# slcs-jsc/mptrac

Hardware: AMD Instinct MI355X
Metric: particle-steps/s (higher is better)
Workload: dtype f64

## Files before the change

### mptrac_amd/csrc/mphip_api.hip

```cpp
#include <hip/hip_runtime.h>
#include <dlfcn.h>
#include <unistd.h>

#include <algorithm>
#include <atomic>
#include <cmath>
#include <cstdio>
#include <cstring>
#include <string>
#include <mutex>
#include <thread>
#include <vector>

#include "mphip_kernels.hpp"
#include "mphip_metprep.hpp"

using namespace mphip;

namespace {

constexpr unsigned kAdv = MPHIP_MOD_TIMESTEPS | MPHIP_MOD_POSITION | MPHIP_MOD_ADVECT | MPHIP_MOD_POSITION2;
constexpr unsigned kAdvTurb = kAdv | MPHIP_MOD_DIFF_TURB;
constexpr unsigned kAdvDiff = kAdvTurb | MPHIP_MOD_DIFF_MESO;
constexpr unsigned kAdvTurbConvSedi = kAdvTurb | MPHIP_MOD_CONVECTION | MPHIP_MOD_SEDI;
constexpr unsigned kAdvDiffConvSedi = kAdvDiff | MPHIP_MOD_CONVECTION | MPHIP_MOD_SEDI;
constexpr unsigned kDiffConvSediOnly = MPHIP_MOD_TIMESTEPS | MPHIP_MOD_DIFF_TURB | MPHIP_MOD_DIFF_MESO | MPHIP_MOD_CONVECTION
  | MPHIP_MOD_SEDI | MPHIP_MOD_POSITION2;
constexpr unsigned kTailOnly = MPHIP_MOD_TIMESTEPS;
constexpr unsigned kBound = MPHIP_MOD_BOUND_COND | MPHIP_MOD_BOUND_COND2;
constexpr unsigned kParticleBits = 0x3fffu | MPHIP_MOD_ISOSURF | kBound | MPHIP_MOD_ISOSURF_INIT;

struct MetSlot {
  bool valid = false;
  double time = 0;
  float *f3[MPHIP_N3D] = {};
  float *f2[MPHIP_N2D] = {};
  bool has3[MPHIP_N3D] = {};
  bool has2[MPHIP_N2D] = {};
  std::vector<double> lon, lat, p;
  float ps11 = 0.f;
  double ps_min = -HUGE_VAL, pct_min = -HUGE_VAL;
  double ps_max = HUGE_VAL, pbl_min = -HUGE_VAL, pbl_max = HUGE_VAL, pel_min = -HUGE_VAL;
};

}

struct mphip_ctx {
  int device = 0;
  hipStream_t stream = nullptr;
  std::string err;
  std::mutex err_lock;

  mphip_ctl_t ctl;
  bool have_ctl = false;
  DevClim *d_clim = nullptr;
  bool have_clim = false;
  double *d_zm[MPHIP_NZM] = {};
  DevZm zm[MPHIP_NZM] = {};
  double *d_ts[MPHIP_NTR] = {};
  DevTracerSeries h_tracers = {};
  DevTracerSeries *d_tracers = nullptr;

  MetSlot slot[2];
  int flip = 0;
  MetSlot next;
  bool next_pending = false;
  hipStream_t copy_stream = nullptr;
  hipEvent_t next_ready = nullptr;
  hipEvent_t main_mark = nullptr;
  bool fuse_sort = true;
  const int *fused_perm = nullptr;
  bool fuse_quantities = true;
  bool fused_quantities = false;
  bool lazy_meteo = true;
  bool meteo_pending = false;
  bool pin_host_atm = false;
  std::vector<std::pair<uintptr_t, uintptr_t>> pinned;
  std::mutex pinned_lock;
  std::thread uploader;
  int uploader_rc = 0;
  std::atomic<bool> uploader_done{ false };
  std::string uploader_err;
  int nx = 0, ny = 0, npl = 0, coord_type = 0;
  int nml = 0;
  struct PackedGrids {
    float *wind = nullptr, *temp = nullptr, *h2o = nullptr;
    float *mlw = nullptr, *zl2 = nullptr, *pl2 = nullptr;
    f32x4 *mx = nullptr, *mx2 = nullptr;
    f32x4 *cloud = nullptr, *sfa = nullptr, *sfb = nullptr, *sfc = nullptr, *sfd = nullptr;
    f32x4 *cp2 = nullptr;
    int *ml_mono = nullptr;
    bool ml_monotonic = false;
    void release() {
      for (void *q : { (void *) wind, (void *) temp, (void *) h2o, (void *) mlw, (void *) zl2, (void *) pl2, (void *) mx,
                       (void *) mx2, (void *) cloud, (void *) sfa, (void *) sfb, (void *) sfc, (void *) sfd, (void *) cp2,
                       (void *) ml_mono })
        if (q)
          (void) hipFree(q);
      *this = PackedGrids();
    }
  };
  PackedGrids pk, pk_next;
  bool pk_next_valid = false;
  std::vector<double> h_lon, h_lat, h_p;
  double *d_axes = nullptr;
  int lut_base = 0, lut_size = 0;
  size_t axes_bytes = 0;
  bool packed_dirty = true;

  long long np = 0, ip0 = 0, np_total = 0, cap = 0;
  int nq = 0;
  double *d_arr[4 + MPHIP_NQ_MAX] = {};
  double *d_alt[4 + MPHIP_NQ_MAX] = {};
  float *d_uvwp[3] = {};
  float *d_uvwp_alt[3] = {};
  double *d_dt = nullptr;
  double *d_dt_alt = nullptr;
  uint64_t rng_ctr = 0;
  double *d_iso = nullptr, *d_iso_alt = nullptr;
  int *d_kz = nullptr, *d_kz_alt = nullptr;
  double *d_iso_ts = nullptr, *d_iso_ps = nullptr;
  int iso_n = 0;

  int *d_ext = nullptr, *d_ext_alt = nullptr;
  bool ext_identity = true;
  int locality_interval = 60;
  double *d_rec = nullptr;
  size_t rec_cap = 0;
  bool grid_records = true;
  int chain_blocks = 0;
  double *h_sums = nullptr;
  size_t h_sums_cap = 0;
  double *d_grid_kernel = nullptr;
  double *d_ana_kernel = nullptr;
  size_t ana_kernel_cap = 0;
  uint32_t *d_marks = nullptr;
  size_t marks_cap = 0;
  int *d_slot_of = nullptr;
  size_t slot_of_cap = 0;
  uint32_t *d_ana_flags = nullptr;
  int grid_nk = 0;
  bool locality_zorder = false;
  int locality_tile = 0;
  int step_blocks = 8192;
  int step_blocks_multi = 32768;
  int xcd_map = 1;
  int big_grid = 0;
  int perm_records = 1;
  void *d_prec = nullptr;
  size_t prec_cap = 0;
  int multi_step = 64;
  bool force_generic = false;
  bool compact_depo = true;
  int sort_bits = 0;
  int steps_since_resort = 1 << 30;

  uint32_t *d_keys[2] = {};
  int *d_vals[2] = {};
  uint32_t *d_counts = nullptr;
  size_t counts_cap = 0;
  int sorted_buf = -1;
  int lds_tile = 0;
  bool emit_keys = true;
  unsigned char *d_depo_busy = nullptr;
  long long depo_busy_cap = 0;
  bool depo_busy_valid = false;
  bool sort_repair = true;
  bool ahead_priority = false;
  bool stored_is_sorted = false;
  long long sorted_n = 0;
  uint32_t *rep_sk = nullptr, *rep_mk[2] = {}, *rep_fk = nullptr, *rep_tiles = nullptr, *rep_nm = nullptr;
  int *rep_si = nullptr, *rep_mi[2] = {}, *rep_fv = nullptr;
  long long rep_cap = 0;
  bool sort_ahead = true;
  bool ahead_box = true;
  hipStream_t ahead_stream = nullptr;
  hipEvent_t ahead_mark = nullptr, ahead_done = nullptr;
  uint32_t *ahead_keys[2] = {};
  int *ahead_vals[2] = {};
  uint32_t *ahead_counts = nullptr;
  size_t ahead_counts_cap = 0;
  double *ahead_dt = nullptr;
  long long ahead_cap = 0;
  bool ahead_valid = false;
  double ahead_t = 0;
  int ahead_cur = 0;

  int *d_cell = nullptr;
  double *d_sums = nullptr;
  size_t sums_cap = 0;

  int *d_cnt = nullptr;
  double *d_chemgrid = nullptr;
  bool chemgrid_ok = false;
  double h2o2_low = 0;
  double *d_photo = nullptr;
  DevPhoto photo = {};
  bool photo_have[4] = {};
  RadioQnt radio = { { -1, -1, -1, -1, -1, -1 } };
  bool radio_on = false;
  bool rdepo_on = false;
  mphip_box_t rdepo_grid = {};
  double *d_rdepo_inv = nullptr;
  size_t rdepo_ntot = 0;
  bool rdepo_have_t = false;
  double rdepo_t = 0;
  const unsigned char *depo_busy_last = nullptr;
  unsigned depo_busy_last_mask = 0;
  bool mix_exchange_levels = false;
  double *d_occ = nullptr, *h_occ = nullptr, *d_band = nullptr;
  int *d_band_cnt = nullptr;
  size_t band_cap = 0;
  int mix_band_lo = -1, mix_band_hi = -1;
  size_t cnt_cap = 0;
  int deterministic_sums = 1;
  int sum_path = 0;
  unsigned long long *d_lists = nullptr;
  size_t lists_cap = 0;

  mphip_allreduce_fn allreduce = nullptr;
  void *allreduce_user = nullptr;
  void *comm = nullptr;
  int comm_ranks = 1, comm_rank = 0;

  std::mutex prep_lock;
  hipStream_t prep_stream = nullptr;
  int prep_nx = 0, prep_ny = 0, prep_np = 0;
  float *prep_in3[MPHIP_N3D] = {}, *prep_in2[MPHIP_N2D] = {};
  float *prep_out2[MPHIP_N2D] = {};
  float *prep_z[2] = {};
  double *prep_axes = nullptr;
  int prep_profile_phase = 0;

  bool prof = false;
  std::vector<hipEvent_t> ev;
  size_t ev_used = 0;
};

namespace {

int fail(mphip_ctx *ctx, const std::string &msg) {
  if (ctx) {
    std::lock_guard<std::mutex> guard(ctx->err_lock);
    ctx->err = msg;
  }
  return 1;
}

#define HIPCHK(call)                                                                         \
  do {                                                                                       \
    hipError_t e_ = (call);                                                                  \
    if (e_ != hipSuccess)                                                                    \
      return fail(ctx, std::string(#call) + ": " + hipGetErrorString(e_));                   \
  } while (0)

template <typename T>
int dev_alloc(mphip_ctx *ctx, T **p, size_t n) {
  if (*p) {
    HIPCHK(hipFree(*p));
    *p = nullptr;
  }
  if (n) {
    HIPCHK(hipMalloc((void **) p, n * sizeof(T)));
  }
  return 0;
}

void dev_free(void *p) {
  if (p)
    (void) hipFree(p);
}

int grid_for(long long n, int block = 256, int maxb = 8192) {
  long long b = (n + block - 1) / block;
  if (b < 1)
    b = 1;
  if (b > maxb)
    b = maxb;
  return (int) b;
}

DevAtm dev_atm(const mphip_ctx *c) {
  DevAtm a;
  a.time = c->d_arr[0];
  a.p = c->d_arr[1];
  a.lon = c->d_arr[2];
  a.lat = c->d_arr[3];
  for (int iq = 0; iq < MPHIP_NQ_MAX; iq++)
    a.q[iq] = iq < c->nq ? c->d_arr[4 + iq] : nullptr;
  a.up = c->d_uvwp[0];
  a.vp = c->d_uvwp[1];
  a.wp = c->d_uvwp[2];
  a.dt = c->d_dt;
  a.ext = c->ext_identity ? nullptr : c->d_ext;
  a.iso = c->d_iso;
  a.kz = c->d_kz;
  a.iso_ts = c->d_iso_ts;
  a.iso_ps = c->d_iso_ps;
  a.iso_n = c->iso_n;
  a.perm = c->fused_perm;
  a.s_time = c->d_alt[0];
  a.s_p = c->d_alt[1];
  a.s_lon = c->d_alt[2];
  a.s_lat = c->d_alt[3];
  a.nq_perm = c->fused_perm && c->fused_quantities ? c->nq : 0;
  for (int iq = 0; iq < MPHIP_NQ_MAX; iq++)
    a.s_q[iq] = iq < c->nq ? c->d_alt[4 + iq] : nullptr;
  a.np = c->np;
  a.ip0 = c->ip0;
  a.np_total = c->np_total;
  return a;
}

DevMet dev_met(const mphip_ctx *c) {
  DevMet M;
  M.wind = c->pk.wind;
  M.temp = c->pk.temp;
  M.cloud = c->pk.cloud;
  M.mx = c->pk.mx;
  M.mx2 = c->pk.mx2;
  M.sfa = c->pk.sfa;
  M.sfb = c->pk.sfb;
  M.cp2 = c->pk.cp2;
  M.sfc = c->pk.sfc;
  M.sfd = c->pk.sfd;
  M.h2o = c->pk.h2o;
  M.mlw = c->pk.mlw;
  M.zl2 = c->pk.zl2;
  M.pl2 = c->pk.pl2;
  M.ml_monotonic = c->pk.ml_monotonic ? 1 : 0;
  for (int t = 0; t < 2; t++) {
    M.zl[t] = c->slot[t ^ c->flip].f3[MPHIP_ZETAL];
    M.pll[t] = c->slot[t ^ c->flip].f3[MPHIP_PL];
  }
  M.npl = c->nml;
  M.axes = c->d_axes;
  M.lut_base = c->lut_base;
  M.lut_size = c->lut_size;
  M.lat_x0 = c->h_lat[0];
  M.lat_inv_dx = (c->ny - 1) / (c->h_lat[c->ny - 1] - c->h_lat[0]);
  M.nx = c->nx;
  M.ny = c->ny;
  M.np = c->npl;
  M.coord_type = c->coord_type;
  M.time0 = c->slot[0 ^ c->flip].time;
  M.time1 = c->slot[1 ^ c->flip].time;
  M.inv_dtime = 1.0 / (M.time1 - M.time0);
  double latmin = c->h_lat[0], latmax = c->h_lat[0];
  for (double v : c->h_lat) {
    latmin = std::min(latmin, v);
    latmax = std::max(latmax, v);
  }
  M.latmin = latmin;
  M.latmax = latmax;
  M.local = (std::fabs(c->h_lon[c->nx - 1] - c->h_lon[0] - 360.0) >= 0.01);
  const int my = (c->ny - 1) >> 1, mp = (c->npl - 1) >> 1;
  M.lat_ascending = c->h_lat[my] < c->h_lat[my + 1];
  M.p_ascending = c->h_p[mp] < c->h_p[mp + 1];
  M.lon_first = c->h_lon[0];
  M.lon_last = c->h_lon[c->nx - 1];
  M.inv_dlon0 = 1.0 / (c->h_lon[1] - c->h_lon[0]);
  M.lat_search_max = std::nextafter(latmax, -HUGE_VAL);
  M.p_min = *std::min_element(c->h_p.begin(), c->h_p.end());
  M.p_search_max = std::nextafter(*std::max_element(c->h_p.begin(), c->h_p.end()), -HUGE_VAL);
  M.p_cmp_off = M.p_ascending ? 1 : 0;
  M.p_step = M.p_ascending ? 1 : -1;
  M.ps11[0] = c->slot[0 ^ c->flip].ps11;
  M.ps11[1] = c->slot[1 ^ c->flip].ps11;
  M.ps_skip = std::min(c->slot[0].ps_min, c->slot[1].ps_min) - 1e-6;
  M.pct_skip = std::min(c->slot[0].pct_min, c->slot[1].pct_min) - 1e-6;
  {
    const double ps_lo = std::min(c->slot[0].ps_min, c->slot[1].ps_min), ps_hi = std::max(c->slot[0].ps_max, c->slot[1].ps_max);
    const double pbl_lo = std::min(c->slot[0].pbl_min, c->slot[1].pbl_min),
                 pbl_hi = std::max(c->slot[0].pbl_max, c->slot[1].pbl_max);
    auto p1_min = [&](double trans) {
      double lo = HUGE_VAL;
      for (double pbl : { pbl_lo, pbl_hi })
        for (double ps : { ps_lo, ps_hi })
          lo = std::min(lo, pbl - trans * (ps - pbl));
      return lo;
    };
    const bool known = std::isfinite(ps_lo) && std::isfinite(ps_hi) && std::isfinite(pbl_lo) && std::isfinite(pbl_hi);
    M.turb_skip = -HUGE_VAL;
    M.conv_skip = -HUGE_VAL;
    if (known && c->have_ctl) {
      const double b = std::min({ ps_lo, pbl_lo, p1_min(c->ctl.turb_pbl_trans) });
      M.turb_skip = b - 1e-6 * std::fabs(b) - 1e-6;
      double lo = ps_lo;
// ... 1028 lines not shown
  int cur = 0, rc = 0;
  if (box && !keys_ready)
    rc = sort_keys(ctx, 0, &t_next, box);
  if (!rc && (hipEventRecord(ctx->ahead_mark, main_stream) != hipSuccess
              || hipStreamWaitEvent(ctx->ahead_stream, ctx->ahead_mark, 0) != hipSuccess))
    rc = fail(ctx, "stream hand-over of the sort ahead of time failed");
  ctx->stream = ctx->ahead_stream;
  if (!rc && !box && !keys_ready)
    rc = sort_keys(ctx, 0, &t_next, nullptr);
  if (!rc)
    rc = key_prev ? repair_sort(ctx, key_prev, n, bits_for(sort_key_range(ctx, 0)), &cur)
                  : radix_passes(ctx, ctx->d_keys, ctx->d_vals, n, bits_for(sort_key_range(ctx, 0)), &cur, nullptr, true);
  ctx->stream = main_stream;
  ahead_swap_buffers(ctx);
  if (rc)
    return 1;
  HIPCHK(hipEventRecord(ctx->ahead_done, ctx->ahead_stream));
  ctx->ahead_valid = true;
  ctx->ahead_t = t_next;
  ctx->ahead_cur = cur;
  return 0;
}

int permute_random(mphip_ctx *ctx, const PermArgs &g, const int *index, long long n, bool scatter) {
  const PermGeom pg = perm_geom(n);
  RecordGeom rg;
  rg.n8 = g.n8;
  rg.n4 = g.n4;
  const int words4 = g.n4 + (g.ext_out ? 1 : 0);
  rg.chunks = (g.n8 + 1) / 2 + (words4 + 3) / 4;
  rg.inv = 65536 / rg.chunks + 1;
  for (int p = 0; p < 64 * rg.chunks; p++)
    if ((int) (((unsigned) p * (unsigned) rg.inv) >> 16) != p / rg.chunks)
      return fail(ctx, "internal: record piece index");
  const size_t need = (size_t) n * (size_t) rg.chunks * 16;
  bool records = ctx->perm_records && n >= 65536;
  if (records && need > ctx->prec_cap) {
    if (ctx->d_prec)
      (void) hipFree(ctx->d_prec);
    ctx->d_prec = nullptr;
    ctx->prec_cap = 0;
    if (hipMalloc(&ctx->d_prec, need) == hipSuccess)
      ctx->prec_cap = need;
    else {
      (void) hipGetLastError();
      records = false;
    }
  }
  if (!records) {
    if (scatter)
      hipLaunchKernelGGL(perm_scatter_kernel, dim3(pg.nblocks), dim3(256), 0, ctx->stream, g, index, n, pg);
    else
      hipLaunchKernelGGL(perm_gather_kernel, dim3(pg.nblocks), dim3(256), 0, ctx->stream, g, index, n, pg);
    HIPCHK(hipGetLastError());
    return 0;
  }
  f32x4u *rec = (f32x4u *) ctx->d_prec;
  const size_t lds = (size_t) kRecordWaves * 64 * (size_t) rg.chunks * 16;
  hipLaunchKernelGGL(perm_pack_kernel, dim3(pg.nblocks), dim3(64 * kRecordWaves), lds, ctx->stream, g, rg,
                     scatter ? index : (const int *) nullptr, rec, n, pg);
  hipLaunchKernelGGL(perm_unpack_kernel, dim3(pg.nblocks), dim3(64 * kRecordWaves), lds, ctx->stream, g, rg,
                     scatter ? (const int *) nullptr : index, (const f32x4u *) rec, n, pg);
  HIPCHK(hipGetLastError());
  return 0;
}

int restore_external_order(mphip_ctx *ctx) {
  if (ctx->ext_identity || ctx->np == 0) {
    ctx->ext_identity = true;
    return 0;
  }
  if (ahead_drop(ctx))
    return 1;
  PermArgs g = perm_args(ctx, true);
  if (permute_random(ctx, g, ctx->d_ext, ctx->np, true))
    return 1;
  perm_swap(ctx, true);
  ctx->stored_is_sorted = false;
  ctx->ext_identity = true;
  ctx->steps_since_resort = 1 << 30;
  return 0;
}

int locality_sort(mphip_ctx *ctx) {
  if (ctx->np == 0)
    return 0;
  if (ahead_drop(ctx) || ensure_packed(ctx))
    return 1;
  int cur = 0;
  const int tile = ctx->locality_tile > 0 ? ctx->locality_tile : (ctx->have_ctl && ml_winds(ctx->ctl) ? 8 : 4);
  if (sort_pairs(ctx, tile, &cur, nullptr))
    return 1;
  PermArgs g = perm_args(ctx, true);
  g.ext_in = ctx->ext_identity ? nullptr : ctx->d_ext;
  g.ext_out = ctx->d_ext_alt;
  if (ctx->ext_identity) {
    if (permute_random(ctx, g, ctx->d_vals[cur], ctx->np, false))
      return 1;
  } else {
    const PermGeom pg = perm_geom(ctx->np);
    hipLaunchKernelGGL(perm_gather_kernel, dim3(pg.nblocks), dim3(256), 0, ctx->stream, g, ctx->d_vals[cur], ctx->np, pg);
    HIPCHK(hipGetLastError());
  }
  perm_swap(ctx, true);
  std::swap(ctx->d_ext, ctx->d_ext_alt);
  ctx->stored_is_sorted = false;
  ctx->ext_identity = false;
  ctx->steps_since_resort = 0;
  return 0;
}

int do_sort(mphip_ctx *ctx, const double *timestep_t = nullptr) {
  const long long n = ctx->np;
  if (n == 0)
    return 0;
  int cur = 0;
  if (timestep_t && ctx->ahead_valid && ctx->ahead_t == *timestep_t && ctx->ext_identity) {
    HIPCHK(hipStreamWaitEvent(ctx->stream, ctx->ahead_done, 0));
    ahead_swap_buffers(ctx);
    ctx->ahead_valid = false;
    cur = ctx->ahead_cur;
  } else {
    if (ahead_drop(ctx) || ensure_packed(ctx) || restore_external_order(ctx))
      return 1;
    if (sort_pairs(ctx, 0, &cur, timestep_t))
      return 1;
  }
  ctx->sorted_buf = cur;
  ctx->stored_is_sorted = true;
  ctx->sorted_n = n;
  const PermGeom pg = perm_geom(n);
  if (timestep_t && ctx->fuse_sort) {
    PermArgs g;
    memset(&g, 0, sizeof(g));
    g.n8 = ctx->nq;
    for (int k = 0; k < ctx->nq; k++) {
      g.in8[k] = ctx->d_arr[4 + k];
      g.out8[k] = ctx->d_alt[4 + k];
    }
    ctx->fused_quantities = ctx->fuse_quantities;
    if (ctx->nq > 0 && !ctx->fused_quantities) {
      hipLaunchKernelGGL(perm_gather_kernel, dim3(pg.nblocks), dim3(256), 0, ctx->stream, g, ctx->d_vals[cur], n, pg);
      HIPCHK(hipGetLastError());
    }
    for (int k = 0; k < 4 + ctx->nq; k++)
      std::swap(ctx->d_arr[k], ctx->d_alt[k]);
    ctx->fused_perm = ctx->d_vals[cur];
  } else {
    PermArgs g = perm_args(ctx, false);
    hipLaunchKernelGGL(perm_gather_kernel, dim3(pg.nblocks), dim3(256), 0, ctx->stream, g, ctx->d_vals[cur], n, pg);
    HIPCHK(hipGetLastError());
    perm_swap(ctx, false);
  }
  ctx->steps_since_resort = 0;
  return 0;
}

int ensure_sums(mphip_ctx *ctx, size_t n) {
  if (n > ctx->sums_cap) {
    if (dev_alloc(ctx, &ctx->d_sums, n))
      return 1;
    ctx->sums_cap = n;
  }
  return 0;
}

struct Rccl {
  typedef struct { char internal[128]; } UniqueId;
  int (*GetUniqueId)(UniqueId *) = nullptr;
  int (*CommInitRank)(void **, int, UniqueId, int) = nullptr;
  int (*CommDestroy)(void *) = nullptr;
  int (*AllReduce)(const void *, void *, size_t, int, int, void *, hipStream_t) = nullptr;
  int (*GroupStart)() = nullptr;
  int (*GroupEnd)() = nullptr;
  int (*CommCount)(void *, int *) = nullptr;
  int (*CommUserRank)(void *, int *) = nullptr;
  const char *(*GetErrorString)(int) = nullptr;
  bool ok = false;
  std::string why;
};
constexpr int kNcclInt32 = 2, kNcclFloat64 = 8, kNcclSum = 0;

Rccl &rccl() {
  static Rccl r;
  static std::once_flag once;
  std::call_once(once, [] {
    void *h = nullptr;
    for (const char *name : { "librccl.so.1", "librccl.so", "/opt/rocm/lib/librccl.so.1" })
      if ((h = dlopen(name, RTLD_NOW | RTLD_GLOBAL)))
        break;
    if (!h) {
      r.why = std::string("cannot load librccl.so: ") + dlerror();
// ... 2019 lines not shown
  bool emitted = false;
  if (sort_next && ctx->ahead_box && ctx->emit_keys) {
    MixPlan plan;
    bool act = false;
    if (mixing_plan(ctx, t, &plan, &act) || ahead_ensure(ctx))
      return 1;
    if (act) {
      ek.keys = ctx->ahead_keys[0];
      ek.dt_next = ctx->ahead_dt;
      ek.cell = ctx->d_cell;
      ek.grid = plan.box.grid;
      ek.box_t0 = plan.box.t0;
      ek.box_t1 = plan.box.t1;
      ek.ens = plan.box.ens;
      ek.ngrid = plan.box.ngrid;
      ek.direction = (double) c.direction;
      ek.t_start = c.t_start;
      ek.t_stop = c.t_stop;
      ek.t_next = t_next;
      constexpr unsigned kDepo = MPHIP_MOD_WET_DEPO | MPHIP_MOD_DRY_DEPO;
#ifndef MPHIP_DEPO_FLAGS
#define MPHIP_DEPO_FLAGS 1
#endif
      if (MPHIP_DEPO_FLAGS && (tail & kDepo) && !(tail & ~kDepo) && ctx->compact_depo) {
        if (ctx->np > ctx->depo_busy_cap) {
          if (dev_alloc(ctx, &ctx->d_depo_busy, (size_t) ctx->np))
            return 1;
          ctx->depo_busy_cap = ctx->np;
        }
        ek.depo_busy = ctx->d_depo_busy;
        ek.depo_mask = tail;
      }
    }
  }
  if (launch_step(ctx, mask, t, P.rng, 1, 0, 0, &ek, &emitted))
    return 1;
  bool cells_ready = false;
  if (sort_next) {
    MixPlan plan;
    if (mixing_plan(ctx, t, &plan, &cells_ready))
      return 1;
    const BoxArgs box = { ctx->d_cell, plan.box.grid, plan.box.t0, plan.box.t1, plan.box.ens, plan.box.ngrid };
    if (!ctx->ahead_box)
      cells_ready = false;
    if (ahead_launch(ctx, t_next, cells_ready ? &box : nullptr, emitted && cells_ready))
      return 1;
  }
  if (do_mixing(ctx, t, cells_ready))
    return 1;
  if (chem && launch_chem(ctx, t))
    return 1;
  if (tail && launch_step(ctx, tail, t))
    return 1;
  if (rdepo && radio_depo_step())
    return 1;
  return P.due.meteo ? schedule_meteo(ctx) : 0;
}

int mphip_run_timesteps(mphip_ctx *ctx, double t_first, int nsteps) {
  if (!ctx)
    return 1;
  if (!ctx->have_ctl)
    return fail(ctx, "control parameters were not uploaded");
  if (nsteps < 0)
    return fail(ctx, "mphip_run_timesteps: negative step count");
  const mphip_ctl_t &c = ctx->ctl;
  const double stride = c.direction * c.dt_mod;
  double t = t_first;
  int done = 0;
  while (done < nsteps) {
    int batch = 0;
    const bool meteo = meteo_requested(c);
    auto meteo_at = [&](double tt) { return meteo && due_at(c, tt).meteo; };
    auto scheduled = [&](double tt) {
      const StepDue d = due_at(c, tt);
      return d.sort || d.mixing || (d.conv && c.conv_dt > 0);
    };
    const bool quiet = ctx->multi_step && ctx->np > 0 && t != c.t_start && !scheduled(t)
      && c.advect > 0
      && !ctx->fused_perm
      && !ctx->force_generic
      && !step_chem_on(c)
      && !step_radio_depo_on(ctx);
    if (quiet) {
      batch = nsteps - done;
      if (ctx->locality_interval > 0)
        batch = std::min(batch, ctx->locality_interval - ctx->steps_since_resort);
      batch = std::min(batch, ctx->multi_step);
      double tt = t;
      for (int j = 0; j < batch; j++) {
        if (j > 0 && scheduled(tt)) {
          batch = j;
          break;
        }
        const double tn = tt + stride;
        if (meteo_at(tt) && (!ctx->lazy_meteo || !meteo_at(tn))) {
          batch = j + 1;
          break;
        }
        tt = tn;
      }
    }
    StepPlan P{};
    if (batch > 1) {
      HIPCHK(hipSetDevice(ctx->device));
      if (ensure_packed(ctx))
        return 1;
      P = plan_step(ctx, t);
      if (step_kernel_mask(ctx, P.mask | P.tail, batch) == kNoStepKernel || (ml_winds(c) && !ctx->d_kz))
        batch = 1;
    }
    if (batch < 2) {
      if (mphip_run_timestep(ctx, t))
        return 1;
      t += stride;
      done++;
      continue;
    }
    if (settle_meteo(ctx, meteo_at(t)))
      return 1;
    if (launch_step(ctx, P.mask | P.tail, t, P.rng, batch, stride, P.per_step))
      return 1;
    ctx->rng_ctr += P.per_step * (uint64_t) batch;
    if (ctx->steps_since_resort < (1 << 29))
      ctx->steps_since_resort += batch;
    double t_last = t;
    for (int k = 0; k < batch; k++) {
      t_last = t;
      t += stride;
    }
    done += batch;
    if (meteo_at(t_last) && schedule_meteo(ctx))
      return 1;
  }
  return 0;
}

int mphip_module(mphip_ctx *ctx, unsigned modules, double t) {
  if (ctx && ahead_drop(ctx))
    return 1;
  if (!ctx)
    return 1;
  if (!ctx->have_ctl)
    return fail(ctx, "control parameters were not uploaded");
  HIPCHK(hipSetDevice(ctx->device));
  if (flush_meteo(ctx))
    return 1;
  switch (modules) {
  case MPHIP_MOD_SORT:
    return do_sort(ctx);
  case MPHIP_MOD_MIXING:
    return do_mixing(ctx, t);
  case MPHIP_MOD_METEO:
    return launch_meteo(ctx);
  case MPHIP_MOD_OH_CHEM:
    return launch_oh(ctx);
  case MPHIP_MOD_CHEM_GRID:
    return do_chem_grid(ctx, t);
  case MPHIP_MOD_H2O2_CHEM:
    return launch_h2o2(ctx);
  case MPHIP_MOD_TRACER_CHEM:
    return launch_tracer_chem(ctx);
  case MPHIP_MOD_RADIO_DEPO:
    return launch_radio_depo(ctx, t, nullptr);
  }
  if (modules & MPHIP_MOD_RADIO_DECAY) {
    modules &= ~(unsigned) MPHIP_MOD_RADIO_DECAY;
    if (radio_any(ctx))
      modules |= kRadioDecay;
    else if (!modules)
      return 0;
  }
  if (modules & ~(kParticleBits | kRadioDecay))
    return fail(ctx, "module_sort / module_mixing / module_meteo / module_chem_grid / module_oh_chem / module_h2o2_chem "
                     "/ module_tracer_chem / module_radio_depo must be called on their own");
  uint64_t per_step = 0;
  const RngCtr rng = rng_counters(modules, (uint64_t) ctx->np_total, ctx->rng_ctr, &per_step);
  ctx->rng_ctr += per_step;
  if (modules & MPHIP_MOD_TIMESTEPS)
    modules |= kStoreDt;
  return launch_step(ctx, modules, t, rng);
}

int mphip_get_sort(mphip_ctx *ctx, double *keys, int *perm) {
  if (!ctx || ctx->sorted_buf < 0)
    return fail(ctx, "module_sort has not been run");
  HIPCHK(hipSetDevice(ctx->device));
  const long long n = ctx->np;
  if (perm)
    HIPCHK(hipMemcpyAsync(perm, ctx->d_vals[ctx->sorted_buf], (size_t) n * sizeof(int), hipMemcpyDeviceToHost,
                          ctx->stream));
  if (keys) {
    double *d_tmp = nullptr;
    HIPCHK(hipMalloc((void **) &d_tmp, (size_t) n * sizeof(double)));
    hipLaunchKernelGGL(keys_to_double_kernel, dim3(grid_for(n)), dim3(256), 0, ctx->stream,
                       ctx->d_keys[ctx->sorted_buf], d_tmp, n);
    HIPCHK(hipMemcpyAsync(keys, d_tmp, (size_t) n * sizeof(double), hipMemcpyDeviceToHost, ctx->stream));
    HIPCHK(hipStreamSynchronize(ctx->stream));
    HIPCHK(hipFree(d_tmp));
  }
  HIPCHK(hipStreamSynchronize(ctx->stream));
  return 0;
}

// ... 537 lines not shown
}

int mphip_comm_init(mphip_ctx *ctx, int nranks, int rank, const void *id128) {
  if (!ctx || !id128 || nranks < 1 || rank < 0 || rank >= nranks)
    return fail(ctx, "bad communicator arguments");
  Rccl &R = rccl();
  if (!R.ok)
    return fail(ctx, R.why);
  HIPCHK(hipSetDevice(ctx->device));
  if (ctx->comm) {
    HIPCHK(hipStreamSynchronize(ctx->stream));
    RCCLCHK(R.CommDestroy(ctx->comm));
    ctx->comm = nullptr;
  }
  Rccl::UniqueId id;
  memcpy(&id, id128, sizeof(id));
  StdoutToStderr quiet;
  RCCLCHK(R.CommInitRank(&ctx->comm, nranks, id, rank));
  ctx->comm_ranks = nranks;
  ctx->comm_rank = rank;
  return 0;
}

int mphip_comm_destroy(mphip_ctx *ctx) {
  if (!ctx)
    return 1;
  if (ctx->comm) {
    HIPCHK(hipSetDevice(ctx->device));
    HIPCHK(hipStreamSynchronize(ctx->stream));
    RCCLCHK(rccl().CommDestroy(ctx->comm));
    ctx->comm = nullptr;
  }
  ctx->comm_ranks = 1;
  ctx->comm_rank = 0;
  return 0;
}

int mphip_comm_query(mphip_ctx *ctx, int *nranks, int *rank) {
  if (!ctx || !nranks || !rank)
    return 1;
  *nranks = 0;
  *rank = 0;
  if (!ctx->comm)
    return 0;
  Rccl &R = rccl();
  RCCLCHK(R.CommCount(ctx->comm, nranks));
  RCCLCHK(R.CommUserRank(ctx->comm, rank));
  return 0;
}

int mphip_set_option(mphip_ctx *ctx, const char *name, double value) {
  if (!ctx || !name)
    return 1;
  if (strcmp(name, "locality_sort_interval") == 0) {
    if (value < 0)
      return fail(ctx, "locality_sort_interval must be >= 0");
    ctx->locality_interval = (int) value;
    return 0;
  }
  if (strcmp(name, "step_blocks") == 0 || strcmp(name, "step_blocks_multi") == 0) {
    if (value < 8 || value > 1048576)
      return fail(ctx, "step_blocks must be in 8 ... 1048576");
    (strcmp(name, "step_blocks") == 0 ? ctx->step_blocks : ctx->step_blocks_multi) = (int) value;
    return 0;
  }
  if (strcmp(name, "fuse_sort") == 0) {
    ctx->fuse_sort = value != 0;
    return 0;
  }
  if (strcmp(name, "lazy_meteo") == 0) {
    if (value == 0 && flush_meteo(ctx))
      return 1;
    ctx->lazy_meteo = value != 0;
    return 0;
  }
  if (strcmp(name, "pin_host_atm") == 0) {
    ctx->pin_host_atm = value != 0;
    return 0;
  }
  if (strcmp(name, "multi_step") == 0) {
    if (value < 0 || value > 4096)
      return fail(ctx, "multi_step must be in 0 ... 4096");
    ctx->multi_step = (int) value;
    return 0;
  }
  if (strcmp(name, "fuse_sort_quantities") == 0) {
    ctx->fuse_quantities = value != 0;
    return 0;
  }
  if (strcmp(name, "perm_records") == 0) {
    ctx->perm_records = value != 0;
    return 0;
  }
  if (strcmp(name, "big_grid") == 0) {
    ctx->big_grid = value != 0;
    return 0;
  }
  if (strcmp(name, "derive_profile_phase") == 0) {
    if (value != 0 && value != 1 && value != 2)
      return fail(ctx, "derive_profile_phase must be 0 (kernels), 1 (uploads) or 2 (downloads)");
    ctx->prep_profile_phase = (int) value;
    return 0;
  }
  if (strcmp(name, "xcd_map") == 0) {
    ctx->xcd_map = value != 0;
    return 0;
  }
  if (strcmp(name, "generic_kernel") == 0) {
    ctx->force_generic = value != 0;
    return 0;
  }
  if (strcmp(name, "sort_bits") == 0) {
    if (!(value == 0 || (value >= 8 && value <= kRadixMaxBits)))
      return fail(ctx, "sort_bits must be 0 (automatic), 8, 9 or 10");
    ctx->sort_bits = (int) value;
    return 0;
  }
  if (strcmp(name, "mix_exchange_levels") == 0) {
    ctx->mix_exchange_levels = value != 0;
    return 0;
  }
  if (strcmp(name, "lds_tile") == 0) {
    if (value != 0 && (value < 64 || value > 2400))
      return fail(ctx, "lds_tile must be 0 or 64 ... 2400 cells");
    ctx->lds_tile = (int) value;
    return 0;
  }
  if (strcmp(name, "ahead_priority") == 0) {
    ctx->ahead_priority = value != 0;
    return 0;
  }
  if (strcmp(name, "emit_keys") == 0) {
    ctx->emit_keys = value != 0;
    return 0;
  }
  if (strcmp(name, "sort_repair") == 0) {
    ctx->sort_repair = value != 0;
    return 0;
  }
  if (strcmp(name, "compact_depo") == 0) {
    ctx->compact_depo = value != 0;
    return 0;
  }
  if (strcmp(name, "ahead_box") == 0) {
    ctx->ahead_box = value != 0;
    return 0;
  }
  if (strcmp(name, "sort_ahead") == 0) {
    if (ahead_drop(ctx))
      return 1;
    ctx->sort_ahead = value != 0;
    return 0;
  }
  if (strcmp(name, "sum_path") == 0) {
    if (!(value == 0 || value == 1 || value == 2))
      return fail(ctx, "sum_path must be 0, 1 or 2");
    ctx->sum_path = (int) value;
    return 0;
  }
  if (strcmp(name, "deterministic_sums") == 0) {
    if (!(value == 0 || value == 1))
      return fail(ctx, "deterministic_sums must be 0 or 1");
    ctx->deterministic_sums = (int) value;
    return 0;
  }
  if (strcmp(name, "grid_records") == 0) {
// ... 176 lines not shown
```

### mptrac_amd/csrc/mphip_device.hpp

```cpp
#pragma once

#include <hip/hip_runtime.h>
#include <stdint.h>

#pragma GCC visibility push(default)
#include "../../include/mptrac_hip.h"
#pragma GCC visibility pop
#include "mphip_libm.h"
#include "mphip_libmtab.h"

namespace mphip {

struct LibmBlob {
  double log_tab[2 * MPHIP_LIBM_N];
  uint64_t exp_tab[2 * MPHIP_LIBM_N];
  double pow_tab[3 * MPHIP_LIBM_N];
};
static __device__ const LibmBlob g_libm = { { MPHIP_LIBM_LOG_TAB_INIT }, { MPHIP_LIBM_EXP_TAB_INIT }, { MPHIP_LIBM_POW_TAB_INIT } };
constexpr int kLibmLogExpDoubles = 4 * MPHIP_LIBM_N;
constexpr int kLibmDoubles = 7 * MPHIP_LIBM_N;

__device__ __forceinline__ const double *libm_tables() {
  return g_libm.log_tab;
}
// ... 44 lines not shown
__device__ __forceinline__ double libm_cos_wide(double x) {
  int handled;
  const double r = mphip_libm_cos_wide(g_sincos_tab, x, &handled);
  return handled ? r : cos(x);
}

__device__ __forceinline__ double libm_sin_wide(double x) {
  int handled;
  const double r = mphip_libm_sin_wide(g_sincos_tab, x, &handled);
  return handled ? r : sin(x);
}

typedef float f32x4 __attribute__((ext_vector_type(4)));

constexpr double kG0 = 9.80665;
constexpr double kH0 = 7.0;
constexpr double kKB = 1.3806504e-23;
constexpr double kMA = 28.9644;
constexpr double kP0 = 1013.25;
constexpr double kRI = 8.3144598;
constexpr double kRA = 1e3 * kRI / kMA;
constexpr double kRE = 6367.421;
constexpr double kMAir = 4.8096e-26;
constexpr double kTRef = 298.15;
constexpr double kT0 = 273.15;
constexpr double kPi = 3.14159265358979323846;
constexpr double kSO2K1Ref = 1.23e-2, kSO2K1Temp = 2.01e3, kSO2K2Ref = 6e-8, kSO2K2Temp = 1.12e3;
constexpr double kWdTLiquid = kT0, kWdTIce = 238.15, kWdTLiquidBC = 270.;
constexpr double kEps = 18.01528 / kMA, kKappa = 0.286, kCpd = 1003.5, kKarman = 0.40;


struct DevMet {
  const float *wind;
  const float *temp;
  const f32x4 *cloud;
  const f32x4 *mx;
  const f32x4 *mx2;
  const f32x4 *sfa;
  const f32x4 *sfb;
  const f32x4 *cp2;
  const f32x4 *sfc;
  const f32x4 *sfd;
  const float *h2o;
  const float *mlw;
  const float *zl[2];
  const float *pll[2];
  const float *zl2, *pl2;
  int ml_monotonic;
  int npl;
  const double *axes;
  int nx, ny, np, coord_type;
  int lut_base, lut_size;
  double lat_x0, lat_inv_dx;
  double time0, time1;
  double inv_dtime;
  double latmin, latmax;
  int local;
  int lat_ascending, p_ascending;
  double lon_first, lon_last;
  double inv_dlon0;
  double lat_search_max;
  double p_min, p_search_max;
  int p_cmp_off, p_step;
  float ps11[2];
  double ps_skip, pct_skip;
  double turb_skip, conv_skip;
  double meso_dt, meso_r, meso_r2;
};

struct DevAtm {
  double *time, *p, *lon, *lat;
  double *q[MPHIP_NQ_MAX];
  float *up, *vp, *wp;
  double *dt;
  const int *ext;
  double *iso;
  int *kz;
  const double *iso_ts, *iso_ps;
  int iso_n;
  const int *perm;
  const double *s_time, *s_p, *s_lon, *s_lat;
  const double *s_q[MPHIP_NQ_MAX];
  int nq_perm;
  long long np;
  long long ip0;
  long long np_total;
};

struct DevClim {
  int ntime, nlat;
  double time[12];
  double lat[73];
  double tropo[12][73];
  double inv_dtime[12];
  double inv_dlat[73];
};

struct Axes {
  const double *lon, *lat, *p;
  const double *inv_lon, *inv_lat, *inv_p;
  const short *p_lut;
};

__device__ __forceinline__ size_t axes_doubles(const DevMet &M) {
  return 2 * (size_t) (M.nx + M.ny + M.np);
}

__device__ __forceinline__ Axes load_axes(const DevMet &M, double *smem) {
  const size_t nd = axes_doubles(M);
  for (size_t i = threadIdx.x; i < nd; i += blockDim.x)
    smem[i] = M.axes[i];
  short *lut = (short *) (smem + nd);
  const short *glut = (const short *) (M.axes + nd);
  for (int i = threadIdx.x; i < M.lut_size; i += blockDim.x)
    lut[i] = glut[i];
  Axes A;
  A.lon = smem;
  A.lat = A.lon + M.nx;
  A.p = A.lat + M.ny;
  A.inv_lon = A.p + M.np;
  A.inv_lat = A.inv_lon + M.nx;
  A.inv_p = A.inv_lat + M.ny;
  A.p_lut = lut;
  return A;
}

#ifndef MPHIP_EXACT_DIV
#define MPHIP_EXACT_DIV 0
#endif
#ifndef MPHIP_WIND_CACHE
#define MPHIP_WIND_CACHE 1
#endif
#ifndef MPHIP_SETPRIO
#define MPHIP_SETPRIO 0
#endif


__device__ __forceinline__ double div_const(double x, double y, double inv_y) {
#if MPHIP_EXACT_DIV
  (void) inv_y;
  return x / y;
#else
  (void) y;
  return x * inv_y;
#endif
}


__device__ __forceinline__ double fdiv(double a, double b) {
#if MPHIP_EXACT_DIV
  return a / b;
#else
  double r = __builtin_amdgcn_rcp(b);
  r = __builtin_fma(__builtin_fma(-b, r, 1.0), r, r);
  const double q = a * r;
  return __builtin_fma(__builtin_fma(-b, q, a), r, q);
#endif
}

__device__ __forceinline__ double fsqrt(double x) {
#if MPHIP_EXACT_DIV
  return sqrt(x);
#else
  const double y = __builtin_amdgcn_rsq(x);
  double g = x * y, h = 0.5 * y;
  const double r = __builtin_fma(-h, g, 0.5);
// ... 2996 lines not shown
```

### mptrac_amd/csrc/mphip_kernels.hpp

```cpp
#pragma once

#include <type_traits>
#include "mphip_device.hpp"

namespace mphip {



struct BoxGrid {
  double lon0, lon1, lat0, lat1, z0, z1;
  int nx, ny, nz;
};

constexpr int kMixMax = 8 + MPHIP_NRADIO;
struct MixSet {
  double *q[kMixMax];
  int n;
};

__device__ __forceinline__ int box_cell(const BoxGrid &G, double t0, double t1, double time, double lon, double lat,
                                        double p, const double *__restrict__ ens, long long i, int ngrid) {
  const double dz = (G.z1 - G.z0) / G.nz;
  const double dlon = (G.lon1 - G.lon0) / G.nx;
  const double dlat = (G.lat1 - G.lat0) / G.ny;
// ... 415 lines not shown
  E.dt_next[i] = dt;
  Stencil s;
  raw_cell_fast(M, A, P.lon, P.lat, P.p, s);
  E.keys[i] = (uint32_t) ((s.ix * M.ny + s.iy) * M.np + s.ip);
}

struct RngEarly {
  unsigned mask;
  uint64_t ctr_turb, ctr_meso, ctr_conv, g;
  const double *ltab;
  double turb[3], meso[3], conv;
  double e, o;
  __device__ __forceinline__ void pair_of(uint64_t c0, int which, double *out) {
    const uint64_t i0 = 3 * g;
    const uint64_t y = (c0 + (i0 & ~1ull)) * kSquaresKey;
    if (which == 0) {
      normal_pair_from(ltab, y, e, o);
      pin(e);
      pin(o);
    } else {
      double eb, ob;
      normal_pair_from(ltab, y + 2 * kSquaresKey, eb, ob);
      const bool odd = (i0 & 1) != 0;
      out[0] = odd ? o : e;
      out[1] = odd ? eb : o;
      out[2] = odd ? ob : eb;
      pin(out[0]);
      pin(out[1]);
      pin(out[2]);
    }
  }
  __device__ __forceinline__ void operator()(int stage) {
#if MPHIP_RNG_BALANCED
    if (stage < 2 && (mask & MPHIP_MOD_DIFF_TURB))
      pair_of(ctr_turb, stage, turb);
    if (stage >= 2 && (mask & MPHIP_MOD_DIFF_MESO))
      pair_of(ctr_meso, stage - 2, meso);
    if (stage == 3 && (mask & MPHIP_MOD_CONVECTION)) {
      conv = uniform01(ctr_conv + g);
      pin(conv);
    }
#else
    if (stage == 0 && (mask & MPHIP_MOD_DIFF_TURB)) {
      normal_triple(ltab, ctr_turb, g, turb[0], turb[1], turb[2]);
      pin(turb[0]);
      pin(turb[1]);
      pin(turb[2]);
    }
    if (stage == 1 && (mask & MPHIP_MOD_DIFF_MESO)) {
      normal_triple(ltab, ctr_meso, g, meso[0], meso[1], meso[2]);
      pin(meso[0]);
      pin(meso[1]);
      pin(meso[2]);
    }
    if (stage == 2 && (mask & MPHIP_MOD_CONVECTION)) {
      conv = uniform01(ctr_conv + g);
      pin(conv);
    }
#endif
  }
};
#ifndef MPHIP_MULTI_KEEP_WIND
#define MPHIP_MULTI_KEEP_WIND 0
#endif
#ifndef MPHIP_MULTI_WAVES_PER_SIMD
#define MPHIP_MULTI_WAVES_PER_SIMD 4
#endif
#ifndef MPHIP_SPLITB_WAVES_PER_SIMD
#define MPHIP_SPLITB_WAVES_PER_SIMD 4
#endif
#ifndef MPHIP_ML_OFF32
#define MPHIP_ML_OFF32 1
#endif
#ifndef MPHIP_ML_WAVES_PER_SIMD
#define MPHIP_ML_WAVES_PER_SIMD 3
#endif
#ifndef MPHIP_PBL_WAVES_PER_SIMD
#define MPHIP_PBL_WAVES_PER_SIMD 4
#endif
constexpr bool step_kernel_parks(unsigned ct) {
  return ct < kMaskGenericMLMulti && (ct & kMultiStep) && !(ct & (kMLWinds | kPblClosure))
    && (ct & (MPHIP_MOD_DIFF_TURB | MPHIP_MOD_DIFF_MESO | MPHIP_MOD_CONVECTION | MPHIP_MOD_SEDI));
}
constexpr int kParkDoubles = 256 * 2 + 128;
constexpr size_t kParkBytes = kParkDoubles * sizeof(double);
enum { kParkRp = 0, kParkRhop = 256, kParkExt = 512 };
template <class T>
__device__ __forceinline__ T *park_slot(double *area, int slot, long long i) {
  unsigned lane = (unsigned) i & 255u;
  asm volatile("" : "+v"(lane));
  return (T *) (area + slot) + lane;
}

template <unsigned CT>
__global__ __launch_bounds__(256, kLeanML<CT> ? MPHIP_ML_WAVES_PER_SIMD : !kRuntimeMask<CT> && (CT & kPblClosure) ? MPHIP_PBL_WAVES_PER_SIMD : !kRuntimeMask<CT> ? ((CT & kMultiStep) ? MPHIP_MULTI_WAVES_PER_SIMD
                                                        : (CT & MPHIP_MOD_ADVECT) || CT == MPHIP_MOD_TIMESTEPS ? MPHIP_LEAN_WAVES_PER_SIMD : MPHIP_SPLITB_WAVES_PER_SIMD)
                                   : (CT == kMaskGenericPL ? MPHIP_STEP_WAVES_PER_SIMD : MPHIP_GENERIC_WAVES_PER_SIMD)) void step_kernel(
  const StepParams S) {
  extern __shared__ double s_lds[];
  constexpr bool park = step_kernel_parks(CT);
  double *const s_axes = s_lds + (park ? kParkDoubles : 0);
  const unsigned mask = kRuntimeMask<CT> ? S.mask : (CT & ~kTemplateFlags);
  using MLCol = std::conditional_t<kLeanML<CT> && MPHIP_ML_OFF32 && !kBig<CT>, uint32_t, size_t>;
  const DevMet &M = S.met;
  const DevAtm &a = S.atm;
  const mphip_ctl_t &ctl = S.ctl;

  const Axes A = load_axes(M, s_axes);
  const DevClim *clim = S.clim;
  if ((mask | (kRuntimeMask<CT> ? 0u : (S.mask & kTailModules))) & (MPHIP_MOD_DIFF_TURB | MPHIP_MOD_DECAY)) {
    double *dst = s_axes + ((axes_doubles(M) * 8 + (size_t) M.lut_size * 2 + 15) & ~(size_t) 15) / 8;
    const double *src = (const double *) S.clim;
    for (int i = threadIdx.x; i < (int) (sizeof(DevClim) / sizeof(double)); i += blockDim.x)
      dst[i] = src[i];
    clim = (const DevClim *) dst;
  }
  const double *ltab = libm_tables();
  if (!kRuntimeMask<CT> && (mask & (MPHIP_MOD_DIFF_TURB | MPHIP_MOD_DIFF_MESO | MPHIP_MOD_SEDI))) {
    double *dst = s_axes + ((axes_doubles(M) * 8 + (size_t) M.lut_size * 2 + 15) & ~(size_t) 15) / 8
      + sizeof(DevClim) / sizeof(double);
    const double *src = libm_tables();
    for (int i = threadIdx.x; i < ((CT & kPblClosure) ? kLibmDoubles : kLibmLogExpDoubles); i += blockDim.x)
      dst[i] = src[i];
    ltab = dst;
  }
  __syncthreads();

  long long first, last;
  block_range(S, a.np, first, last);

  for (long long i = first + threadIdx.x; i < last; i += (park ? 256 : blockDim.x)) {
#if MPHIP_PARAMS_RELOAD
    auto kp = (const __attribute__((address_space(4))) StepParams *) __builtin_amdgcn_kernarg_segment_ptr();
    asm volatile("" : "+s"(kp));
    const StepParams &S = *(const StepParams *) kp;
    const DevMet &M = S.met;
    const DevAtm &a = S.atm;
    const mphip_ctl_t &ctl = S.ctl;
#endif
    constexpr bool multi = (!kRuntimeMask<CT> && (CT & kMultiStep) != 0) || CT == kMaskGenericMLMulti;
    const int nsteps = multi ? S.nsteps : 1;
    double t_now = S.t;
    uint64_t c_turb = S.ctr_turb, c_meso = S.ctr_meso, c_conv = S.ctr_conv, c_pbl = S.ctr_pbl;
    constexpr bool store_once = multi && !kRuntimeMask<CT> && !kModelLevels<CT>;
    Particle P;
    WindCache wc;
    float up = 0.f, vp = 0.f, wp = 0.f;
    for (int step = 0; step < nsteps; step++, t_now += S.t_stride, c_turb += S.ctr_stride, c_meso += S.ctr_stride,
             c_conv += S.ctr_stride, c_pbl += S.ctr_stride) {
    const bool fused_sort = a.perm != nullptr;
    if (!multi || step == 0) {
    if (fused_sort) {
      const long long src = a.perm[i];
      P.time = a.s_time[src];
      P.lon = a.s_lon[src];
      P.lat = a.s_lat[src];
      P.p = a.s_p[src];
      for (int k = 0; k < a.nq_perm; k++)
        a.q[k][i] = a.s_q[k][src];
    } else {
      P.time = ld_state(&a.time[i]);
      P.lon = ld_state(&a.lon[i]);
      P.lat = ld_state(&a.lat[i]);
      P.p = ld_state(&a.p[i]);
    }
    if (multi) {
      if (MPHIP_MULTI_KEEP_WIND)
        wind_cache_reset(wc, true);
      if (mask & MPHIP_MOD_DIFF_MESO) {
        up = ld_state(&a.up[i]);
        vp = ld_state(&a.vp[i]);
        wp = ld_state(&a.wp[i]);
      }
    }
    if constexpr (park) {
      if (a.ext)
        *park_slot<int>(s_lds, kParkExt, i) = ld_state(&a.ext[i]);
      if (((CT & kGated) ? mask & S.mask : mask) & MPHIP_MOD_SEDI) {
        *park_slot<double>(s_lds, kParkRp, i) = ld_state(&a.q[ctl.qnt_rp][i]);
        *park_slot<double>(s_lds, kParkRhop, i) = ld_state(&a.q[ctl.qnt_rhop][i]);
      }
    }
    }
    if (CT == kMaskGeneric && (mask & (MPHIP_MOD_ADVECT_INIT | MPHIP_MOD_ISOSURF_INIT))) {
      P.dt = 0;
      if (mask & MPHIP_MOD_ISOSURF_INIT)
        a.iso[i] = isosurf_value(ctl, M, A, P);
      if (mask & MPHIP_MOD_ADVECT_INIT)
        a.p[i] = pressure_from_zeta(M, A, P.time, a.q[ctl.qnt_zeta][i], P.lon, P.lat);
      continue;
    }
    if (kModelLevels<CT> && (mask & MPHIP_MOD_ADVECT_INIT)) {
      a.p[i] = pressure_from_zeta_fast(M, A, P.time, a.q[ctl.qnt_zeta][i], P.lon, P.lat);
      continue;
    }
    if (S.mask & MPHIP_MOD_TIMESTEPS) {
      P.dt = timestep_of(ctl, M, A, P.time, P.lon, P.lat, t_now);
      if (S.mask & kStoreDt)
        a.dt[i] = P.dt;
    } else
      P.dt = a.dt[i];
    if (P.dt == 0) {
      if (fused_sort && !store_once) {
        a.time[i] = P.time;
        a.lon[i] = P.lon;
        a.lat[i] = P.lat;
        a.p[i] = P.p;
      }
      if (CT == kMaskGeneric && (mask & MPHIP_MOD_ISOSURF))
        a.p[i] = isosurf_pressure(ctl, M, A, a, P, ctl.isosurf <= 3 ? a.iso[i] : 0.0);
      if constexpr (!kRuntimeMask<CT> && (CT & kEmitKeys) != 0)
        if (S.emit.keys)
          emit_sort_keys(S.emit, ctl, M, A, i, P);
      if constexpr (!kRuntimeMask<CT> && (CT & kPblClosure) != 0)
        if (S.mask & MPHIP_MOD_ISOSURF) {
          P.p = isosurf_call(&ctl, &M, A, &a, P.time, P.p, P.lon, P.lat, ctl.isosurf <= 3 ? a.iso[i] : 0.0);
          if (!store_once)
            a.p[i] = P.p;
        }
      continue;
    }
    const uint64_t g_held = park ? 0 : (uint64_t) (a.ip0 + (a.ext ? (long long) ld_state(&a.ext[i]) : i));
    auto g_now = [&]() -> uint64_t {
      if constexpr (park)
        return (uint64_t) (a.ip0 + (a.ext ? (long long) *park_slot<int>(s_lds, kParkExt, i) : i));
      else
        return g_held;
    };

    constexpr bool early = MPHIP_RNG_EARLY && !kRuntimeMask<CT> && (CT & MPHIP_MOD_ADVECT) && !(CT & kTwoStage) && !kLeanML<CT>;
    RngEarly pre;
    pre.mask = mask;
    pre.ctr_turb = c_turb;
    pre.ctr_meso = c_meso;
    pre.ctr_conv = c_conv;
    pre.g = early ? g_now() : 0;
    pre.ltab = ltab;

    constexpr bool lean = !kRuntimeMask<CT>;
    if (!kModelLevels<CT> && !(multi && MPHIP_MULTI_KEEP_WIND))
      wind_cache_reset(wc, CT != kMaskGeneric && (lean || !MPHIP_EXACT_DIV));
    if (mask & MPHIP_MOD_POSITION) {
      if (lean)
        position_fast(M, A, P);
      else
        position(M, A, P);
    }
    if (mask & MPHIP_MOD_ADVECT) {
      if (CT == kMaskGeneric && ctl.advect_vert_coord == 2) {
        advect_mlp(ctl, M, A, P);
      } else if (kModelLevels<CT> && ctl.advect_vert_coord == 2) {
        int kz = a.kz[i];
        advect_mlp_fast<MLCol>(ctl, M, A, P, kz);
        a.kz[i] = kz;
      } else if (CT == kMaskGeneric && (ctl.advect_vert_coord == 1 || ctl.advect_vert_coord == 3)) {
        const int qnt = ctl.advect_vert_coord == 1 ? ctl.qnt_zeta : ctl.qnt_eta;
        double zeta;
        advect_ml(ctl, M, A, P, zeta);
        a.q[qnt][i] = zeta;
// ... 2644 lines not shown
```

Before: 13.83 billion.

## Fold periodic locality resort permutation into the multi-step kernel's first load

Result: faster. 13.99 billion, median of 6 (+1.1%).

```diff
diff --git a/mptrac_amd/csrc/mphip_api.hip b/mptrac_amd/csrc/mphip_api.hip
--- a/mptrac_amd/csrc/mphip_api.hip
+++ b/mptrac_amd/csrc/mphip_api.hip
@@ -72,6 +72,7 @@
   const int *fused_perm = nullptr;
   bool fuse_quantities = true;
   bool fused_quantities = false;
+  const int *fold_perm = nullptr;
   bool lazy_meteo = true;
   bool meteo_pending = false;
   bool pin_host_atm = false;
@@ -150,6 +151,7 @@
   void *d_prec = nullptr;
   size_t prec_cap = 0;
   int multi_step = 64;
+  bool fold_resort = true;
   bool force_generic = false;
   bool compact_depo = true;
   int sort_bits = 0;
@@ -298,12 +300,19 @@
   a.iso_ts = c->d_iso_ts;
   a.iso_ps = c->d_iso_ps;
   a.iso_n = c->iso_n;
-  a.perm = c->fused_perm;
+  a.perm = c->fold_perm ? c->fold_perm : c->fused_perm;
   a.s_time = c->d_alt[0];
   a.s_p = c->d_alt[1];
   a.s_lon = c->d_alt[2];
   a.s_lat = c->d_alt[3];
-  a.nq_perm = c->fused_perm && c->fused_quantities ? c->nq : 0;
+  a.nq_perm = c->fold_perm || (c->fused_perm && c->fused_quantities) ? c->nq : 0;
+  a.perm_all = c->fold_perm ? 1 : 0;
+  a.s_up = c->d_uvwp_alt[0];
+  a.s_vp = c->d_uvwp_alt[1];
+  a.s_wp = c->d_uvwp_alt[2];
+  a.s_dt = c->d_dt_alt;
+  a.s_ext = c->d_ext_alt;
+  a.ext_out = c->d_ext;
   for (int iq = 0; iq < MPHIP_NQ_MAX; iq++)
     a.s_q[iq] = iq < c->nq ? c->d_alt[4 + iq] : nullptr;
   a.np = c->np;
@@ -1498,19 +1507,20 @@
   return 0;
 }
 
-int locality_sort(mphip_ctx *ctx) {
-  if (ctx->np == 0)
-    return 0;
+int locality_sort_keys(mphip_ctx *ctx, int *cur) {
   if (ahead_drop(ctx) || ensure_packed(ctx))
     return 1;
-  int cur = 0;
   const int tile = ctx->locality_tile > 0 ? ctx->locality_tile : (ctx->have_ctl && ml_winds(ctx->ctl) ? 8 : 4);
-  if (sort_pairs(ctx, tile, &cur, nullptr))
-    return 1;
+  return sort_pairs(ctx, tile, cur, nullptr);
+}
+
+int locality_sort_apply(mphip_ctx *ctx, int cur, bool fold) {
   PermArgs g = perm_args(ctx, true);
   g.ext_in = ctx->ext_identity ? nullptr : ctx->d_ext;
   g.ext_out = ctx->d_ext_alt;
-  if (ctx->ext_identity) {
+  if (fold) {
+    ctx->fold_perm = ctx->d_vals[cur];
+  } else if (ctx->ext_identity) {
     if (permute_random(ctx, g, ctx->d_vals[cur], ctx->np, false))
       return 1;
   } else {
@@ -1524,6 +1534,13 @@
   ctx->ext_identity = false;
   ctx->steps_since_resort = 0;
   return 0;
+}
+
+int locality_sort(mphip_ctx *ctx) {
+  if (ctx->np == 0)
+    return 0;
+  int cur = 0;
+  return locality_sort_keys(ctx, &cur) || locality_sort_apply(ctx, cur, false);
 }
 
 int do_sort(mphip_ctx *ctx, const double *timestep_t = nullptr) {
@@ -3709,10 +3726,13 @@
       && !ctx->force_generic
       && !step_chem_on(c)
       && !step_radio_depo_on(ctx);
+    const bool fold = quiet && ctx->fold_resort && ctx->locality_interval > 0
+      && ctx->steps_since_resort >= ctx->locality_interval && !ctx->ext_identity
+      && !ml_winds(c) && !ctx->d_iso && !ctx->d_kz && ctx->lds_tile <= 0;
     if (quiet) {
       batch = nsteps - done;
       if (ctx->locality_interval > 0)
-        batch = std::min(batch, ctx->locality_interval - ctx->steps_since_resort);
+        batch = std::min(batch, fold ? ctx->locality_interval : ctx->locality_interval - ctx->steps_since_resort);
       batch = std::min(batch, ctx->multi_step);
       double tt = t;
       for (int j = 0; j < batch; j++) {
@@ -3734,7 +3754,8 @@
       if (ensure_packed(ctx))
         return 1;
       P = plan_step(ctx, t);
-      if (step_kernel_mask(ctx, P.mask | P.tail, batch) == kNoStepKernel || (ml_winds(c) && !ctx->d_kz))
+      const unsigned sel = step_kernel_mask(ctx, P.mask | P.tail, batch);
+      if (sel == kNoStepKernel || (ml_winds(c) && !ctx->d_kz) || (fold && !step_kernel_stores_once(sel)))
         batch = 1;
     }
     if (batch < 2) {
@@ -3746,7 +3767,15 @@
     }
     if (settle_meteo(ctx, meteo_at(t)))
       return 1;
-    if (launch_step(ctx, P.mask | P.tail, t, P.rng, batch, stride, P.per_step))
+    if (fold) {
+      int cur = 0;
+      if (check_fields(ctx, P.mask | P.tail)
+          || locality_sort_keys(ctx, &cur) || locality_sort_apply(ctx, cur, true))
+        return 1;
+    }
+    const int rc = launch_step(ctx, P.mask | P.tail, t, P.rng, batch, stride, P.per_step);
+    ctx->fold_perm = nullptr;
+    if (rc)
       return 1;
     ctx->rng_ctr += P.per_step * (uint64_t) batch;
     if (ctx->steps_since_resort < (1 << 29))
@@ -4450,6 +4479,10 @@
     if (value < 0 || value > 4096)
       return fail(ctx, "multi_step must be in 0 ... 4096");
     ctx->multi_step = (int) value;
+    return 0;
+  }
+  if (strcmp(name, "fold_resort") == 0) {
+    ctx->fold_resort = value != 0;
     return 0;
   }
   if (strcmp(name, "fuse_sort_quantities") == 0) {
diff --git a/mptrac_amd/csrc/mphip_device.hpp b/mptrac_amd/csrc/mphip_device.hpp
--- a/mptrac_amd/csrc/mphip_device.hpp
+++ b/mptrac_amd/csrc/mphip_device.hpp
@@ -150,6 +150,11 @@
   const double *s_time, *s_p, *s_lon, *s_lat;
   const double *s_q[MPHIP_NQ_MAX];
   int nq_perm;
+  int perm_all;
+  const float *s_up, *s_vp, *s_wp;
+  const double *s_dt;
+  const int *s_ext;
+  int *ext_out;
   long long np;
   long long ip0;
   long long np_total;
diff --git a/mptrac_amd/csrc/mphip_kernels.hpp b/mptrac_amd/csrc/mphip_kernels.hpp
--- a/mptrac_amd/csrc/mphip_kernels.hpp
+++ b/mptrac_amd/csrc/mphip_kernels.hpp
@@ -521,6 +521,32 @@
   return ct < kMaskGenericMLMulti && (ct & kMultiStep) && !(ct & (kMLWinds | kPblClosure))
     && (ct & (MPHIP_MOD_DIFF_TURB | MPHIP_MOD_DIFF_MESO | MPHIP_MOD_CONVECTION | MPHIP_MOD_SEDI));
 }
+struct PermRest {
+  float up, vp, wp;
+  int ext;
+};
+__device__ __forceinline__ PermRest perm_rest(const DevAtm &a, long long i, long long src, bool store_uvwp) {
+  PermRest r;
+  a.dt[i] = a.s_dt[src];
+  r.ext = a.s_ext ? a.s_ext[src] : (int) src;
+  a.ext_out[i] = r.ext;
+  r.up = a.s_up[src];
+  r.vp = a.s_vp[src];
+  r.wp = a.s_wp[src];
+  if (store_uvwp) {
+    a.up[i] = r.up;
+    a.vp[i] = r.vp;
+    a.wp[i] = r.wp;
+  }
+  return r;
+}
+__device__ __attribute__((noinline)) PermRest perm_rest_call(const DevAtm *a, long long i, long long src, bool store_uvwp) {
+  return perm_rest(*a, i, src, store_uvwp);
+}
+
+constexpr bool step_kernel_stores_once(unsigned ct) {
+  return ct != 0 && ct < kMaskGenericMLMulti && (ct & kMultiStep) && !(ct & kMLWinds);
+}
 constexpr int kParkDoubles = 256 * 2 + 128;
 constexpr size_t kParkBytes = kParkDoubles * sizeof(double);
 enum { kParkRp = 0, kParkRhop = 256, kParkExt = 512 };
@@ -582,6 +608,7 @@
     double t_now = S.t;
     uint64_t c_turb = S.ctr_turb, c_meso = S.ctr_meso, c_conv = S.ctr_conv, c_pbl = S.ctr_pbl;
     constexpr bool store_once = multi && !kRuntimeMask<CT> && !kModelLevels<CT>;
+    static_assert(store_once == step_kernel_stores_once(CT), "step_kernel_stores_once");
     Particle P;
     WindCache wc;
     float up = 0.f, vp = 0.f, wp = 0.f;
@@ -589,14 +616,29 @@
              c_conv += S.ctr_stride, c_pbl += S.ctr_stride) {
     const bool fused_sort = a.perm != nullptr;
     if (!multi || step == 0) {
+    constexpr bool perm_call = store_once && (CT & kPblClosure) != 0;
+    const bool perm_all = store_once && !perm_call && fused_sort && a.perm_all;
     if (fused_sort) {
       const long long src = a.perm[i];
+      if constexpr (perm_call)
+        if (a.perm_all)
+          (void) perm_rest_call(&a, i, src, true);
       P.time = a.s_time[src];
       P.lon = a.s_lon[src];
       P.lat = a.s_lat[src];
       P.p = a.s_p[src];
       for (int k = 0; k < a.nq_perm; k++)
         a.q[k][i] = a.s_q[k][src];
+      if constexpr (store_once && !perm_call) {
+        if (a.perm_all) {
+          const PermRest r = perm_rest(a, i, src, !(mask & MPHIP_MOD_DIFF_MESO));
+          if constexpr (park)
+            *park_slot<int>(s_lds, kParkExt, i) = r.ext;
+          up = r.up;
+          vp = r.vp;
+          wp = r.wp;
+        }
+      }
     } else {
       P.time = ld_state(&a.time[i]);
       P.lon = ld_state(&a.lon[i]);
@@ -606,14 +648,14 @@
     if (multi) {
       if (MPHIP_MULTI_KEEP_WIND)
         wind_cache_reset(wc, true);
-      if (mask & MPHIP_MOD_DIFF_MESO) {
+      if ((mask & MPHIP_MOD_DIFF_MESO) && !perm_all) {
         up = ld_state(&a.up[i]);
         vp = ld_state(&a.vp[i]);
         wp = ld_state(&a.wp[i]);
       }
     }
     if constexpr (park) {
-      if (a.ext)
+      if (a.ext && !perm_all)
         *park_slot<int>(s_lds, kParkExt, i) = ld_state(&a.ext[i]);
       if (((CT & kGated) ? mask & S.mask : mask) & MPHIP_MOD_SEDI) {
         *park_slot<double>(s_lds, kParkRp, i) = ld_state(&a.q[ctl.qnt_rp][i]);
```
